# typio/entreepy

Measured on AMD Instinct MI355X. Metric: GB/s encode+decode on 1 GiB text at 1/2/4/8 MI355X; % of HBM read peak, higher is better.
Workload: dtype u8; 1 GPU; text-1G: 1073741824 B per GPU, order-0 samples of a_midsummer_nights_dream.txt's byte distribution, seed 0x5EED0004+rank, one step = encode to .et + decode back, HBM-resident; bytes_per_gpu=1073741824, packed_bytes_per_gpu=629699194

## Files before the change

entreepy_amd/csrc/et_api.cpp:

```cpp
#include <sys/stat.h>

#include "et_ctx.h"

#include <algorithm>
#include <cstdlib>
#include <vector>

namespace {

struct Geometry {
    const uint8_t *base;
    uint64_t lo, hi;
    uint32_t rpt, n_tiles;
};

Geometry make_geometry(const et_ctx *ctx, const void *d_text, size_t n) {
    Geometry g;
    const uintptr_t a = reinterpret_cast<uintptr_t>(d_text);
    g.base = reinterpret_cast<const uint8_t *>(a & ~static_cast<uintptr_t>(15));
    g.lo = a & 15;
    g.hi = g.lo + n;
    uint32_t rpt = 1;
    while (rpt < et::MAX_ROUNDS_PER_TILE && g.hi / (static_cast<uint64_t>(rpt) * et::ROUND_BYTES) > 2048) rpt <<= 1;
    if (ctx && ctx->force_rpt) rpt = ctx->force_rpt;
    g.rpt = rpt;
    const uint64_t tile_bytes = static_cast<uint64_t>(rpt) * et::ROUND_BYTES;
    g.n_tiles = static_cast<uint32_t>((g.hi + tile_bytes - 1) / tile_bytes);
    return g;
}

int ensure_encode_ws(et_ctx *ctx, uint32_t n_tiles) {
    ET_TRY(ensure(ctx, ctx->tile_hist, static_cast<size_t>(n_tiles) * 256 * sizeof(uint32_t)));
    ET_TRY(ensure(ctx, ctx->block_hist, static_cast<size_t>(et::MAX_GRID) * 256 * sizeof(uint64_t)));
    ET_TRY(ensure(ctx, ctx->hist, 256 * sizeof(uint64_t)));
    ET_TRY(ensure(ctx, ctx->tile_bits, (static_cast<size_t>(n_tiles) + 1) * sizeof(uint64_t)));
    ET_TRY(ensure(ctx, ctx->tile_off, (static_cast<size_t>(n_tiles) + 1) * sizeof(uint64_t)));
    ET_TRY(ensure(ctx, ctx->enc_table, 768 * sizeof(uint32_t) + HEADER_STAGE));
    ET_TRY(ensure(ctx, ctx->group_sum, (static_cast<size_t>(n_tiles) / 1024 + 2) * sizeof(uint64_t)));
    return ET_OK;
}

float elapsed(et_ctx *ctx, int a, int b) {
    float ms = 0.f;
    if (hipEventElapsedTime(&ms, ctx->ev[a], ctx->ev[b]) != hipSuccess) ms = 0.f;
    return ms;
}

int run_histogram(et_ctx *ctx, const void *d_text, size_t n, const Geometry &g, void *d_hist_also = nullptr) {
    ET_TRY(ensure_encode_ws(ctx, g.n_tiles));
    et::launch_hist(ctx->stream, g.base, g.lo, g.hi, g.rpt, g.n_tiles, static_cast<uint32_t *>(ctx->tile_hist.p),
                    static_cast<unsigned long long *>(ctx->block_hist.p), static_cast<unsigned long long *>(ctx->hist.p),
                    reinterpret_cast<unsigned long long *>(ctx->h_hist), ++ctx->hist_epoch, timed(ctx, 0, 1),
                    static_cast<unsigned long long *>(d_hist_also));
    ET_HIP(hipGetLastError());
    ctx->hist_text = d_text;
    ctx->hist_empty = false;
    ctx->hist_n = n;
    ctx->hist_rpt = g.rpt;
    ctx->hist_tiles = g.n_tiles;
    ctx->hist_on_host = false;
    return ET_OK;
}

int run_body(et_ctx *ctx, const et_codebook *cb, const Geometry &g, uint32_t *out32, uint64_t base_bit,
             const uint8_t *header, size_t header_len, int ev_scan, int ev_body) {
    const bool long_codes = cb->max_length > 32;
    ET_TRY(wait_for_word<uint64_t>(ctx, ctx->h_scalar + 12, ctx->enc_block_epoch, 100.0, "the code table block was never taken"));
    for (int s = 0; s < 256; ++s) {
        const uint32_t len = cb->length[s];
        uint32_t code = cb->data[s];
        if (!long_codes) code = len ? (len == 32 ? code : (code & ((1u << len) - 1u)) << (32 - len)) : 0u;
        ctx->h_enc[2 * s] = code;
        ctx->h_enc[2 * s + 1] = len;
        ctx->h_enc[512 + s] = len;
    }
    const size_t padded = (header_len + 3) & ~static_cast<size_t>(3);
    if (header_len) {
        if (padded > HEADER_STAGE) return fail(ctx, ET_ERR_ARG, "header too long");
        uint8_t *stage = reinterpret_cast<uint8_t *>(ctx->h_enc + 768);
        std::memcpy(stage, header, header_len);
        std::memset(stage + header_len, 0, padded - header_len);
    }
    et::launch_tile_scan(ctx->stream, static_cast<const uint32_t *>(ctx->tile_hist.p), g.n_tiles, cb->length, ctx->h_enc, static_cast<uint32_t *>(ctx->enc_table.p),
                         static_cast<uint32_t>(768 + padded / 4), reinterpret_cast<unsigned long long *>(ctx->h_scalar + 12), ++ctx->enc_block_epoch,
                         static_cast<unsigned long long *>(ctx->tile_bits.p),
                         static_cast<unsigned long long *>(ctx->group_sum.p), scan_epoch(ctx), base_bit,
                         static_cast<unsigned long long *>(ctx->tile_off.p), out32, static_cast<const uint32_t *>(ctx->enc_table.p) + 768,
                         static_cast<uint32_t>(padded / 4));
    ET_HIP(hipGetLastError());
    et::launch_encode(ctx->stream, g.base, g.lo, g.hi, g.rpt, g.n_tiles, static_cast<const unsigned long long *>(ctx->tile_off.p),
                      static_cast<const uint2 *>(ctx->enc_table.p), cb->max_length, out32, timed(ctx, ev_scan, ev_body));
    ET_HIP(hipGetLastError());
    return ET_OK;
}

int fetch_histogram(et_ctx *ctx) {
    if (ctx->hist_on_host) return ET_OK;
    for (uint32_t w = 0; w < et::HIST_REDUCE_GROUPS; ++w)
        ET_TRY(wait_for_word<uint64_t>(ctx, ctx->h_hist + 256 + w, ctx->hist_epoch, 100.0, "the histogram never reached the host"));
    ctx->hist_on_host = true;
    return ET_OK;
}

}

extern "C" const char *et_version(void) { return "entreepy-hip 0.1.0 (gfx950; .et format 0x01, reference v1.1.0)"; }

extern "C" const char *et_last_error(const et_ctx *ctx) { return ctx ? ctx->err.c_str() : ""; }


extern "C" int et_ctx_create(int device, et_ctx **out) {
    if (!out) return ET_ERR_ARG;
    *out = nullptr;
    int count = 0;
    if (hipGetDeviceCount(&count) != hipSuccess || device < 0 || device >= count) return ET_ERR_HIP;
    et_ctx *ctx = new (std::nothrow) et_ctx();
    if (!ctx) return ET_ERR_NOMEM;
    ctx->device = device;
    DeviceGuard guard(device);
    bool ok = guard.ok;
    ok = ok && hipStreamCreateWithFlags(&ctx->own_stream, hipStreamNonBlocking) == hipSuccess;
    ctx->stream = ctx->own_stream;
    ok = ok && hipStreamCreateWithFlags(&ctx->side.stream, hipStreamNonBlocking) == hipSuccess;
    ok = ok && hipEventCreateWithFlags(&ctx->side.fork, hipEventDisableTiming) == hipSuccess;
    ok = ok && hipEventCreateWithFlags(&ctx->side.join, hipEventDisableTiming) == hipSuccess;
    ok = ok && hipEventCreateWithFlags(&ctx->switch_ev, hipEventDisableTiming) == hipSuccess;
    ok = ok && hipHostMalloc(reinterpret_cast<void **>(&ctx->h_hist), (256 + et::HIST_REDUCE_GROUPS) * sizeof(uint64_t)) == hipSuccess;
    if (ok) std::memset(ctx->h_hist, 0, (256 + et::HIST_REDUCE_GROUPS) * sizeof(uint64_t));
    ok = ok && hipHostMalloc(reinterpret_cast<void **>(&ctx->h_enc), 768 * sizeof(uint32_t) + HEADER_STAGE) == hipSuccess;
    ok = ok && hipHostMalloc(reinterpret_cast<void **>(&ctx->h_header), HEADER_STAGE) == hipSuccess;
    for (int i = 0; i < 2; ++i) {
        ok = ok && hipHostMalloc(reinterpret_cast<void **>(&ctx->h_lut_buf[i]), DEC_TABLES_BYTES) == hipSuccess;
    }
    ctx->h_lut = ctx->h_lut_buf[0];
    ok = ok && hipHostMalloc(reinterpret_cast<void **>(&ctx->h_scalar), 16 * sizeof(uint64_t)) == hipSuccess;
    if (ok) std::memset(ctx->h_scalar, 0, 16 * sizeof(uint64_t));
    for (int i = 0; i < 2; ++i) ok = ok && hipHostMalloc(reinterpret_cast<void **>(&ctx->h_tw_tree[i]), sizeof(et::TwUpload)) == hipSuccess;
    for (auto &e : ctx->ev) ok = ok && hipEventCreateWithFlags(&e, hipEventDisableSystemFence) == hipSuccess;
    if (!ok) {
        et_ctx_destroy(ctx);
        return ET_ERR_HIP;
    }
    *out = ctx;
    return ET_OK;
}

extern "C" void et_ctx_destroy(et_ctx *ctx) {
    if (!ctx) return;
    DeviceGuard guard(ctx->device);
    (void)hipStreamSynchronize(ctx->stream);
    DevBuf *bufs[] = {&ctx->tile_hist, &ctx->block_hist, &ctx->hist, &ctx->tile_bits, &ctx->tile_off, &ctx->enc_table, &ctx->group_sum,
                      &ctx->sub_state, &ctx->blk_exit, &ctx->blk_count, &ctx->blk_off, &ctx->lut, &ctx->flag,
                      &ctx->worklist, &ctx->lane_maps, &ctx->blk_maps, &ctx->grp_maps, &ctx->blk_in, &ctx->grp_in, &ctx->row_scratch,
                      &ctx->tw_table, &ctx->tw_tree, &ctx->blk_start, &ctx->blk_pub, &ctx->chain_table, &ctx->io_in, &ctx->io_out};
    for (DevBuf *b : bufs)
        if (b->p) (void)hipFree(b->p);
    delete ctx->io;
    void *pinned[] = {ctx->h_hist, ctx->h_enc, ctx->h_header, ctx->h_lut_buf[0], ctx->h_lut_buf[1], ctx->h_scalar, ctx->h_tw_tree[0], ctx->h_tw_tree[1]};
    for (void *p : pinned)
        if (p) (void)hipHostFree(p);
    for (auto &e : ctx->ev)
        if (e) (void)hipEventDestroy(e);
    if (ctx->own_stream) (void)hipStreamDestroy(ctx->own_stream);
    if (ctx->side.stream) (void)hipStreamDestroy(ctx->side.stream);
    if (ctx->side.fork) (void)hipEventDestroy(ctx->side.fork);
    if (ctx->side.join) (void)hipEventDestroy(ctx->side.join);
    if (ctx->switch_ev) (void)hipEventDestroy(ctx->switch_ev);
    delete ctx;
}

namespace {

int switch_stream(et_ctx *ctx, hipStream_t s) {
    if (s == ctx->stream) return ET_OK;
    DeviceGuard guard(ctx->device);
    ET_HIP(hipEventRecord(ctx->switch_ev, ctx->stream));
    ET_HIP(hipStreamWaitEvent(s, ctx->switch_ev, 0));
    ctx->stream = s;
    return ET_OK;
}

}

extern "C" int et_ctx_set_stream(et_ctx *ctx, void *hip_stream) {
    if (!ctx) return ET_ERR_ARG;
    return switch_stream(ctx, static_cast<hipStream_t>(hip_stream));
}

extern "C" int et_ctx_use_own_stream(et_ctx *ctx) {
    if (!ctx) return ET_ERR_ARG;
    return switch_stream(ctx, ctx->own_stream);
}

extern "C" void *et_ctx_stream(const et_ctx *ctx) { return ctx ? static_cast<void *>(ctx->stream) : nullptr; }

extern "C" int et_ctx_device(const et_ctx *ctx) { return ctx ? ctx->device : -1; }

extern "C" int et_ctx_set_tile_rounds(et_ctx *ctx, uint32_t rounds) {
    if (!ctx) return ET_ERR_ARG;
    if (rounds > et::MAX_ROUNDS_PER_TILE || (rounds & (rounds - 1))) return ET_ERR_ARG;
    ctx->force_rpt = rounds;
    ctx->hist_text = nullptr;
    return ET_OK;
}

extern "C" int et_ctx_enable_timing(et_ctx *ctx, int on) {
    if (!ctx) return ET_ERR_ARG;
    ctx->timing = on != 0 && on != ET_TIMING_DECODE_BODY;
    ctx->timing_body = on == ET_TIMING_DECODE_BODY;
    ctx->pend_enc = ctx->pend_dec = false;
    return ET_OK;
}

extern "C" int et_last_timings_of(et_ctx *ctx, int which, et_timings *out) {
    if (!ctx || !out || which < 0 || which > 1) return ET_ERR_ARG;
    DeviceGuard guard(ctx->device);
    if (which == 0 && ctx->pend_enc) {
        ET_HIP(hipEventSynchronize(ctx->ev[3]));
        if (!ctx->pend_enc_shard) {
            ctx->tm_enc.hist_ms = elapsed(ctx, 0, 1);
            ctx->tm_enc.total_ms = elapsed(ctx, 0, 3);
        }
        ctx->tm_enc.scan_ms = ctx->pend_enc_bits ? elapsed(ctx, 1, 2) : 0.f;
        ctx->tm_enc.body_ms = elapsed(ctx, 2, 3);
        ctx->pend_enc = ctx->pend_enc_shard = false;
    }
    if (which == 1 && ctx->pend_dec && ctx->timing_body) {
        ET_HIP(hipEventSynchronize(ctx->ev[EV_DEC + 3]));
        ctx->tm_dec.body_ms = elapsed(ctx, EV_DEC + 2, EV_DEC + 3);
        ctx->pend_dec = false;
    }
    if (which == 1 && ctx->pend_dec) {
        ET_HIP(hipEventSynchronize(ctx->ev[EV_DEC + 3]));
        ctx->tm_dec.sync_ms = elapsed(ctx, EV_DEC + 0, EV_DEC + 2);
// ... 358 lines not shown
```

entreepy_amd/csrc/et_ctx.h:

```cpp
#pragma once

#include "entreepy_hip.h"

#include "et_io.h"
#include "et_kernels.h"
#include "et_rowsync.h"
#include "et_tables.h"
#include "et_treewalk.h"

#include <hip/hip_runtime.h>

#include <atomic>
#include <chrono>
#include <cstdio>
#include <cstring>
#include <string>

struct DevBuf {
    void *p = nullptr;
    size_t cap = 0;
};

constexpr size_t HEADER_STAGE = 8192;
constexpr size_t SUB_TABLE_ONLY = (static_cast<size_t>(et::DEC_SUB_TABLES_MAX) << et::DEC_SUB_BITS_MAX) * sizeof(uint16_t) + 64;
constexpr size_t SUB_TABLE_BYTES = SUB_TABLE_ONLY + 256;
constexpr size_t DEC_STEPS_OFFSET = (sizeof(uint32_t) << et::DEC_LUT_BITS_MAX) * 2 + 1024 * sizeof(uint32_t) + 2 * SUB_TABLE_BYTES;
constexpr size_t DEC_TABLES_BYTES = DEC_STEPS_OFFSET + (sizeof(uint32_t) << et::DEC_STEP_BITS_MAX) + (sizeof(uint32_t) << et::DEC_LUT_BITS_MAX) +
                                    2 * (et::DEC_STEP_SUB_WORDS + 4) * sizeof(uint32_t) + 2 * sizeof(et::DecodeTables) + sizeof(et::TablePlan) + 64;

enum class Family { TREE_WALK, WINDOWS, ROWS, FIXED_SYNC, FIXED_WRITE, EXIT_MAPS };

struct DecWs {
    uint32_t *sub_state, *blk_exit, *blk_count, *flag, *worklist;
    unsigned long long *blk_off, *group_sum;
};

struct Span : DecWs {
    const uint32_t *words;
    uint64_t n_bytes, n_subs;
    uint32_t n_blocks, first_bit;
    uint32_t tw_mode, dec_flags, row_mode;
    const et_codebook *cb;
    et::RowCode row_code;
    et::DecodeTables tb, tb_write;
    const uint16_t *tw_table;
    uint32_t tw_n_int;
    uint32_t *blk_start, *blk_pub;
    uint32_t *exit_bits;
    const uint64_t *chain;
    uint32_t n_chain;
};

struct et_ctx {
    int device = 0;
    hipStream_t own_stream = nullptr;
    et::SideLane side = {};
    hipStream_t stream = nullptr;
    hipEvent_t switch_ev = nullptr;
    bool timing = false;
    bool timing_body = false;
    uint32_t force_rpt = 0;
    uint32_t lut_bits_write = et::DEC_LUT_BITS_WRITE;
    uint32_t step_bits = et::DEC_STEP_BITS_DEFAULT;
    std::string err;

    DevBuf tile_hist, block_hist, hist, tile_bits, tile_off, enc_table, group_sum;
    DevBuf sub_state, blk_exit, blk_count, blk_off, lut, flag, worklist;
    DevBuf lane_maps, blk_maps, grp_maps, blk_in, grp_in;
    DevBuf row_scratch;
    DevBuf tw_table, tw_tree, blk_start, blk_pub, chain_table;
    et::TwUpload *h_tw_tree[2] = {};
    int tw_turn = 0;
    DevBuf io_in, io_out;
    et_io::Pipe *io = nullptr;

    uint64_t *h_hist = nullptr;
    uint32_t *h_enc = nullptr;
    uint8_t *h_header = nullptr;
    uint32_t *h_lut = nullptr;
    uint32_t *h_lut_buf[2] = {};
    int lut_turn = 0;
    uint64_t *h_scalar = nullptr;

    const void *hist_text = nullptr;
    size_t hist_n = 0;
    uint32_t hist_rpt = 0, hist_tiles = 0;
    bool hist_on_host = false;
    bool hist_empty = false;
    const void *scan_buf = nullptr;
    size_t scan_cap = 0;
    uint32_t scan_epoch_n = 0;
    uint32_t report_epoch = 0;
    uint64_t enc_block_epoch = 0;
    uint64_t header_epoch = 0;
    uint64_t hist_epoch = 0;

    hipEvent_t ev[12] = {};
    et_timings tm_enc = {}, tm_dec = {};
    bool pend_enc = false, pend_dec = false, pend_enc_bits = false, pend_enc_shard = false, pend_dec_first = false;
    int last_kind = 0;
    et_codebook last_cb = {};
    bool have_cb = false;


    struct {
        bool valid = false;
        Family family = Family::WINDOWS;
        Span s = {};
        et_codebook cb = {};
        uint64_t total = 0;
        bool maps_valid = false, maps_const = false;
    } range;
};

struct DeviceGuard {
    int prev = -1;
    bool ok = false;
    explicit DeviceGuard(int dev) {
        if (hipGetDevice(&prev) != hipSuccess) prev = -1;
        ok = hipSetDevice(dev) == hipSuccess;
    }
    ~DeviceGuard() {
        if (prev >= 0) (void)hipSetDevice(prev);
    }
};

inline int fail(et_ctx *ctx, int status, const char *what, hipError_t e = hipSuccess) {
    if (ctx) {
        ctx->err = what;
        if (e != hipSuccess) {
            ctx->err += ": ";
            ctx->err += hipGetErrorString(e);
        }
    }
    return status;
}

#define ET_HIP(call)                                                     \
    do {                                                                 \
        hipError_t e_ = (call);                                          \
        if (e_ != hipSuccess) return fail(ctx, ET_ERR_HIP, #call, e_);   \
    } while (0)

inline int ensure(et_ctx *ctx, DevBuf &b, size_t bytes) {
    if (b.cap >= bytes) return ET_OK;
    if (b.p) {
        ET_HIP(hipStreamSynchronize(ctx->stream));
        ET_HIP(hipFree(b.p));
        b.p = nullptr;
// ... 56 lines not shown
```

entreepy_amd/csrc/et_kernels.h:

```cpp
#pragma once

#include <hip/hip_runtime.h>
#include <stdint.h>

#include "et_tables.h"

#ifdef ET_GUARD_DROP_PINS
#define ET_PIN(x_) ((void)0)
#else
#define ET_PIN(x_) asm volatile("" : "+v"(x_))
#endif

namespace et {

constexpr int BLOCK = 256;
constexpr uint32_t ROUND_BYTES = BLOCK * 16;
constexpr uint32_t MAX_ROUNDS_PER_TILE = 128;
constexpr uint32_t HIST_REDUCE_GROUPS = 128;
constexpr uint32_t MAX_GRID = 2048;

constexpr uint32_t SUB_BITS = 256;
constexpr uint32_t DEC_BLOCK_WORDS = BLOCK * SUB_BITS / 32;
constexpr uint32_t DEC_GUARD_WORDS = 4;
constexpr uint32_t SYNC_CHUNK = 1, WRITE_CHUNK = 4;
constexpr bool SYNC_TICKET = false, WRITE_TICKET = true;
constexpr uint32_t DEC_FIRST_SWEEP_TRIPS = 6;
constexpr uint32_t DEC_REPAIR_SWEEP_TRIPS = 8;
__host__ __device__ inline bool dec_state_final(uint32_t gave_up, uint32_t verify_failed, uint32_t n_blocks) {
    return verify_failed == 0 && static_cast<uint64_t>(gave_up) * 64 <= n_blocks;
}
constexpr uint32_t DEC_HAVE_START = 1, DEC_FRONT_OK = 2;
constexpr uint32_t DEC_SPECIAL_SUPER = 8;
constexpr uint32_t DEC_SPECIAL_ONLY = 4;
constexpr uint32_t DEC_FRONT_WORDS = 4;
constexpr uint32_t DEC_WARMUP_BITS = DEC_FRONT_WORDS * 32;
constexpr uint32_t DEC_STAGED_WORDS = DEC_FRONT_WORDS + DEC_BLOCK_WORDS + DEC_GUARD_WORDS;
constexpr uint32_t DEC_SDATA_WORDS = (DEC_STAGED_WORDS + (DEC_STAGED_WORDS >> 5) + 4) & ~3u;
constexpr uint32_t DEC_STAGE_BYTES = 16384;

struct DecodeTables {
    const uint32_t *lut;
    const uint32_t *longc;
    const uint16_t *sub;
    const uint8_t *sym_len;
    uint32_t lut_bits;
    uint32_t n_long;
    uint32_t sub_bits;
    uint32_t n_sub;
    const uint32_t *steps;
    uint32_t step_bits;
    uint32_t step_sub_bits;
    uint32_t n_step_sub;
    const DecodeTables *dev_copy;
};

struct SideLane {
    hipStream_t stream;
    hipEvent_t fork, join;
};

struct KernelEvents {
    hipEvent_t start = nullptr, stop = nullptr;
};

void launch_hist(hipStream_t stream, const uint8_t *base, uint64_t lo, uint64_t hi, uint32_t rounds_per_tile, uint32_t n_tiles,
                 uint32_t *tile_hist, unsigned long long *block_hist, unsigned long long *hist, unsigned long long *host_hist = nullptr, unsigned long long epoch = 0,
                 KernelEvents ev = {}, unsigned long long *hist_also = nullptr);
__host__ __device__ inline uint32_t header_bound(uint8_t d) { return 8u + 6u * (static_cast<uint32_t>(d) + 1u); }
void launch_words_to_host(hipStream_t stream, const void *d_src, uint32_t n_words, void *host_dst, unsigned long long *host_done, unsigned long long epoch);
void launch_header_to_host(hipStream_t stream, const void *d_src, uint32_t n, void *host_dst, unsigned long long *host_done, unsigned long long epoch);
void launch_tile_scan(hipStream_t stream, const uint32_t *tile_hist, uint32_t n_tiles, const uint8_t *lengths, const uint32_t *host_src, uint32_t *dev_dst,
                      uint32_t copy_words, unsigned long long *host_taken, unsigned long long taken_epoch, unsigned long long *tile_bits, unsigned long long *group_sum, uint32_t epoch, unsigned long long base_bit,
                      unsigned long long *tile_off, uint32_t *out32, const uint32_t *header_src = nullptr, uint32_t header_words = 0);
void launch_encode(hipStream_t stream, const uint8_t *base, uint64_t lo, uint64_t hi, uint32_t rounds_per_tile, uint32_t n_tiles,
                   const unsigned long long *tile_off, const uint2 *enc_table, uint32_t max_len, uint32_t *out32, KernelEvents ev = {});
void launch_dec_sync(hipStream_t stream, const uint32_t *words, uint64_t n_bytes, uint32_t first_bit, uint64_t n_subs,
                     const DecodeTables &tb, uint32_t iter, uint32_t max_trips,
                     uint32_t *sub_state, uint32_t *blk_exit, uint32_t *blk_count, uint32_t *changed, uint32_t *ticket,
                     uint32_t flags = DEC_HAVE_START, uint32_t *worklist = nullptr, uint32_t *n_work = nullptr, const SideLane *side = nullptr,
                     bool ticket_is_zero = false, KernelEvents ev = {});
void launch_dec_maps(hipStream_t stream, const uint32_t *words, uint64_t n_bytes, uint32_t first_bit, bool have_start, uint64_t n_subs,
                     const DecodeTables &tb, uint32_t n_starts, uint32_t map_stride, uint8_t *lane_maps, uint8_t *blk_maps, uint8_t *grp_maps);
void launch_dec_resolve(hipStream_t stream, const uint32_t *words, uint64_t n_bytes, uint32_t first_bit, bool const_first, uint64_t n_subs,
                        const DecodeTables &tb, uint32_t map_stride, const uint8_t *lane_maps, const uint8_t *blk_maps, const uint8_t *grp_maps,
                        uint8_t *blk_in, uint8_t *grp_in, uint32_t *sub_state, uint32_t *blk_exit, uint32_t *blk_count);
void launch_dec_exhaustive(hipStream_t stream, const uint32_t *words, uint64_t n_bytes, uint32_t first_bit, uint64_t n_subs,
                           const DecodeTables &tb, uint32_t n_starts, uint32_t map_stride, uint8_t *lane_maps, uint8_t *blk_maps,
                           uint8_t *grp_maps, uint8_t *blk_in, uint8_t *grp_in, uint32_t *sub_state, uint32_t *blk_exit,
                           uint32_t *blk_count);
void launch_build_dec_tables(hipStream_t stream, const TablePlan *d_plan, uint32_t *lut, uint32_t *longc, uint16_t *sub, uint8_t *sym_len,
                             uint32_t *steps, uint32_t *wsteps, uint32_t *zero16 = nullptr);
void launch_dec_scan(hipStream_t stream, const uint32_t *blk_count, uint32_t n_blocks, unsigned long long *group_sum, uint32_t epoch,
                     unsigned long long *blk_off, unsigned long long *total_copy = nullptr, const uint32_t *verify_state = nullptr,
                     const uint32_t *verify_exit = nullptr, uint32_t *verify_flag = nullptr, uint32_t verify_first = 0xffffffffu,
                     const uint32_t *report_src = nullptr, uint32_t *report_dst = nullptr,
                     bool verify_rows = false,
                     uint32_t report_epoch = 0);
void launch_dec_write(hipStream_t stream, const uint32_t *words, uint64_t n_bytes, uint64_t n_subs, const DecodeTables &tb,
                      const uint32_t *sub_state,
                      const unsigned long long *blk_off, uint64_t n_symbols, uint8_t *out, uint32_t *ticket, const SideLane *side = nullptr,
                      bool ticket_is_zero = false, const uint32_t *void_flags = nullptr, KernelEvents ev = {},
                      const uint64_t *chain = nullptr, uint32_t n_chain = 0, uint32_t chain_max_len = 32,
                      bool strips = false);

}
```

entreepy_amd/csrc/et_kernels.hip:

```cpp
#include "et_kernels_common.h"
#include "et_treewalk.h"

namespace et {

#ifndef ET_NT_LOAD_K1
#define ET_NT_LOAD_K1 1
#endif
#ifndef ET_NT_LOAD_K4
#define ET_NT_LOAD_K4 0
#endif
#ifndef ET_NT_STORE_K4
#define ET_NT_STORE_K4 0
#endif

struct Chunk {
    uint32_t w[4];
    uint32_t valid;
};

__device__ __forceinline__ Chunk load_chunk(const uint8_t *__restrict__ base, uint64_t off, uint64_t lo, uint64_t hi) {
    Chunk c;
    if (off >= lo && off + 16 <= hi) {
        const uint4 v = *reinterpret_cast<const uint4 *>(base + off);
        c.w[0] = v.x; c.w[1] = v.y; c.w[2] = v.z; c.w[3] = v.w;
// ... 78 lines not shown
            uint4 *row = reinterpret_cast<uint4 *>(sh + tid * 32);
#pragma unroll
            for (int q = 0; q < 8; ++q) {
                const int j = (q + tid) & 7;
                const uint4 v = row[j];
                total += v.x + v.y + v.z + v.w;
                row[j] = make_uint4(0, 0, 0, 0);
            }
            tile_hist[static_cast<uint64_t>(t) * 256 + tid] = total;
            acc += total;
        }
        __syncthreads();
    }
    if (tid < 256) block_hist[static_cast<uint64_t>(tid) * HIST_ROWS + blockIdx.x] = acc;
}

__global__ __launch_bounds__(BLOCK) void k_hist_reduce(const unsigned long long *__restrict__ block_hist, uint32_t n_rows,
                                                       unsigned long long *__restrict__ hist, unsigned long long *__restrict__ host_hist,
                                                       unsigned long long epoch, unsigned long long *__restrict__ hist_also) {
    __shared__ unsigned long long part[2][4];
    const int tid = threadIdx.x, lane = tid & 63, wave = tid >> 6;
    const unsigned long long *row0 = block_hist + static_cast<uint64_t>(2 * blockIdx.x) * HIST_ROWS, *row1 = row0 + HIST_ROWS;
    unsigned long long s0 = 0, s1 = 0;
#pragma unroll
    for (uint32_t k = 0; k < HIST_ROWS / BLOCK; ++k) {
        const uint32_t r = k * BLOCK + tid;
        if (r < n_rows) {
            s0 += row0[r];
            s1 += row1[r];
        }
    }
#pragma unroll
    for (int d = 32; d >= 1; d >>= 1) {
        s0 += __shfl_xor(s0, d, 64);
        s1 += __shfl_xor(s1, d, 64);
    }
    if (lane == 0) {
        part[0][wave] = s0;
        part[1][wave] = s1;
    }
    __syncthreads();
    if (tid == 0) {
        const unsigned long long t0 = part[0][0] + part[0][1] + part[0][2] + part[0][3], t1 = part[1][0] + part[1][1] + part[1][2] + part[1][3];
        hist[2 * blockIdx.x] = t0;
        hist[2 * blockIdx.x + 1] = t1;
        if (hist_also) {
            hist_also[2 * blockIdx.x] = t0;
            hist_also[2 * blockIdx.x + 1] = t1;
        }
        if (host_hist) {
            host_hist[2 * blockIdx.x] = t0;
            host_hist[2 * blockIdx.x + 1] = t1;
            __threadfence_system();
            __hip_atomic_store(host_hist + 256 + blockIdx.x, epoch, __ATOMIC_RELEASE, __HIP_MEMORY_SCOPE_SYSTEM);
        }
    }
}

__global__ __launch_bounds__(1024) void k_header_to_host(const uint8_t *__restrict__ src, uint32_t n, uint32_t *__restrict__ host_dst,
                                                         unsigned long long *__restrict__ host_done, unsigned long long epoch) {
    const uint32_t bound = header_bound(255);
    if (bound < n) n = bound;
    for (uint32_t w = threadIdx.x; w * 4 < n; w += 1024) {
        uint32_t v = 0;
        for (uint32_t k = 0; k < 4 && w * 4 + k < n; ++k) v |= static_cast<uint32_t>(src[w * 4 + k]) << (8 * k);
        host_dst[w] = v;
    }
    __threadfence_system();
    __syncthreads();
    if (threadIdx.x == 0) __hip_atomic_store(host_done, epoch, __ATOMIC_RELEASE, __HIP_MEMORY_SCOPE_SYSTEM);
}

__global__ __launch_bounds__(1024) void k_words_to_host(const uint32_t *__restrict__ src, uint32_t n_words, uint32_t *__restrict__ host_dst,
                                                        unsigned long long *__restrict__ host_done, unsigned long long epoch) {
    for (uint32_t w = threadIdx.x; w < n_words; w += 1024) host_dst[w] = src[w];
    __threadfence_system();
    __syncthreads();
    if (threadIdx.x == 0) __hip_atomic_store(host_done, epoch, __ATOMIC_RELEASE, __HIP_MEMORY_SCOPE_SYSTEM);
}

struct CodeLengths {
    uint32_t packed[64];
};
__global__ __launch_bounds__(BLOCK) void k_tile_bits(const uint32_t *__restrict__ tile_hist, uint32_t n_tiles, const CodeLengths lengths,
                                                     unsigned long long *__restrict__ tile_bits, const uint32_t *__restrict__ host_src,
                                                     uint32_t *__restrict__ dev_dst, uint32_t copy_words, unsigned long long *__restrict__ host_taken,
                                                     unsigned long long epoch) {
    const int lane = threadIdx.x & 63;
    if (blockIdx.x == 0) {
        for (uint32_t i0 = threadIdx.x; i0 < copy_words; i0 += 8 * BLOCK) {
            uint32_t v[8];
#pragma unroll
            for (int k = 0; k < 8; ++k) v[k] = i0 + k * BLOCK < copy_words ? host_src[i0 + k * BLOCK] : 0u;
#pragma unroll
            for (int k = 0; k < 8; ++k)
                if (i0 + k * BLOCK < copy_words) dev_dst[i0 + k * BLOCK] = v[k];
        }
        __syncthreads();
        if (threadIdx.x == 0) __hip_atomic_store(host_taken, epoch, __ATOMIC_RELAXED, __HIP_MEMORY_SCOPE_SYSTEM);
    }
    const uint32_t wave_global = blockIdx.x * 4 + (threadIdx.x >> 6), n_waves = gridDim.x * 4;
    const uint32_t l4 = lengths.packed[lane];
    const uint32_t len_x = l4 & 0xffu, len_y = (l4 >> 8) & 0xffu, len_z = (l4 >> 16) & 0xffu, len_w = l4 >> 24;
    for (uint32_t t = wave_global; t < n_tiles; t += n_waves) {
        const uint4 c = reinterpret_cast<const uint4 *>(tile_hist + static_cast<uint64_t>(t) * 256)[lane];
        unsigned long long s = static_cast<unsigned long long>(c.x) * len_x + static_cast<unsigned long long>(c.y) * len_y +
                               static_cast<unsigned long long>(c.z) * len_z + static_cast<unsigned long long>(c.w) * len_w;
#pragma unroll
        for (int d = 32; d >= 1; d >>= 1) s += __shfl_xor(s, d, 64);
        if (lane == 0) tile_bits[t] = s;
    }
}

constexpr unsigned long long SCAN_TOTAL_MASK = (1ull << 47) - 1ull;
constexpr uint32_t SCAN_POLLS = 1u << 22;
template <typename T>
__global__ __launch_bounds__(1024) void k_scan_fused(const T *__restrict__ in, uint32_t n, unsigned long long *__restrict__ out,
                                                     unsigned long long *__restrict__ pub, uint32_t epoch, unsigned long long base,
                                                     uint32_t *__restrict__ zero_words, const uint32_t *__restrict__ header_src, uint32_t header_words,
                                                     unsigned long long *__restrict__ total_copy, const uint32_t *__restrict__ verify_state,
                                                     const uint32_t *__restrict__ verify_exit, uint32_t *__restrict__ verify_flag, uint32_t verify_first,
                                                     uint32_t verify_stride, uint32_t verify_mask, const uint32_t *__restrict__ report_src,
                                                     uint32_t *__restrict__ report_dst, uint32_t report_epoch) {
    __shared__ unsigned long long wsum[16], psum[16];
    __shared__ uint32_t bad_any;
    const int tid = threadIdx.x, lane = tid & 63, wave = tid >> 6;
    const uint32_t g = blockIdx.x, i = g * 1024 + tid;
    if (tid == 0) bad_any = 0;
    __syncthreads();
    if (verify_state && i < n) {
        const uint32_t want = i > 0 ? verify_exit[i - 1] : verify_first;
        if (want != 0xffffffffu && (verify_state[static_cast<uint64_t>(i) * verify_stride] & verify_mask) != want) {
            *verify_flag = 1;
            bad_any = 1;
        }
    }
    const unsigned long long x = (i < n) ? static_cast<unsigned long long>(in[i]) : 0ull;
    const unsigned long long inc = wave_inclusive_scan64(x);
    if (lane == 63) wsum[wave] = inc;
    __syncthreads();
    unsigned long long before = 0;
    for (int w = 0; w < wave; ++w) before += wsum[w];
    const unsigned long long mine = before + inc - x;
    unsigned long long group_total = 0;
    for (int w = 0; w < 16; ++w) group_total += wsum[w];
    const unsigned long long tag = static_cast<unsigned long long>(epoch) << 48;
    if (tid == 0) __hip_atomic_store(pub + g, tag | (bad_any ? 1ull << 47 : 0ull) | (group_total & SCAN_TOTAL_MASK), __ATOMIC_RELAXED, __HIP_MEMORY_SCOPE_AGENT);
    unsigned long long part = 0, bad = 0;
    for (uint32_t j = tid; j < g; j += 1024) {
        unsigned long long v = 0;
        for (uint32_t poll = 0; poll < SCAN_POLLS; ++poll) {
            v = __hip_atomic_load(pub + j, __ATOMIC_RELAXED, __HIP_MEMORY_SCOPE_AGENT);
            if ((v >> 48) == epoch) break;
            __builtin_amdgcn_s_sleep(2);
        }
        part += v & SCAN_TOTAL_MASK;
        bad |= (v >> 47) & 1ull;
    }
#pragma unroll
    for (int d = 32; d >= 1; d >>= 1) {
        part += __shfl_xor(part, d, 64);
        bad |= __shfl_xor(bad, d, 64);
    }
    if (lane == 0) psum[wave] = part | (bad << 63);
    __syncthreads();
    unsigned long long prefix = base;
    bool bad_before = false;
    for (int w = 0; w < 16; ++w) {
        prefix += psum[w] & ~(1ull << 63);
        bad_before = bad_before || (psum[w] >> 63);
    }
    const unsigned long long seam = base >> 5;
    if (i < n) {
        const unsigned long long v = mine + prefix;
        out[i] = v;
        if (zero_words && (i == 0 || ((v & 31) && (v >> 5) != seam))) zero_words[v >> 5] = 0;
    }
    if (g == gridDim.x - 1 && tid == 0) {
        const unsigned long long total = prefix + group_total;
        out[n] = total;
        if (total_copy) *total_copy = total;
        if (zero_words && (total >> 5) != seam && (total & 31)) zero_words[total >> 5] = 0;
        if (report_dst) {
            for (int k = 0; k < 12; ++k) report_dst[k] = report_src[k];
            if (verify_state) report_dst[2] = (bad_before || bad_any) ? 1u : 0u;
            report_dst[12] = static_cast<uint32_t>(total);
            report_dst[13] = static_cast<uint32_t>(total >> 32);
            __threadfence_system();
            __hip_atomic_store(report_dst + 14, report_epoch, __ATOMIC_RELEASE, __HIP_MEMORY_SCOPE_SYSTEM);
        }
    }
    if (g == 0 && header_words) {
        __syncthreads();
        for (uint32_t k = tid; k < header_words; k += 1024) zero_words[k] = header_src[k];
    }
}

struct RingFlush {
    uint32_t *ring;
    uint32_t *out32;
    bool first_word_shared;
};

template <uint32_t RING_WORDS>
__device__ __forceinline__ void flush_words(const RingFlush &f, uint32_t from, uint32_t to) {
    for (uint32_t i = from + threadIdx.x; i < to; i += BLOCK) {
        const uint32_t slot = i & (RING_WORDS - 1);
        const uint32_t v = __builtin_bswap32(f.ring[slot]);
        f.ring[slot] = 0;
        if (i == 0 && f.first_word_shared) atomicOr(f.out32, v);
#if ET_NT_STORE_K4
        else __builtin_nontemporal_store(v, f.out32 + i);
#else
        else f.out32[i] = v;
#endif
    }
}

template <uint32_t RING_WORDS>
__global__ __launch_bounds__(BLOCK) void k_encode_tiles(const uint8_t *__restrict__ base, uint64_t lo, uint64_t hi,
                                                        uint32_t rounds_per_tile, uint32_t n_tiles,
                                                        const unsigned long long *__restrict__ tile_off,
                                                        const uint2 *__restrict__ enc_table, uint32_t *__restrict__ out32) {
    __shared__ __attribute__((aligned(16))) uint32_t ring[RING_WORDS];
    __shared__ __attribute__((aligned(16))) uint2 tab[256];
    __shared__ uint32_t scratch[2][4];
    const int tid = threadIdx.x;
    tab[tid] = enc_table[tid];
    for (uint32_t i = tid; i < RING_WORDS; i += BLOCK) ring[i] = 0;
    __syncthreads();

    const uint64_t tile_bytes = static_cast<uint64_t>(rounds_per_tile) * ROUND_BYTES;
    for (uint32_t t = blockIdx.x; t < n_tiles; t += gridDim.x) {
        const unsigned long long bit0 = tile_off[t];
        RingFlush f;
        f.ring = ring;
        f.out32 = out32 + (bit0 >> 5);
        f.first_word_shared = (bit0 & 31) != 0;
        uint32_t run = static_cast<uint32_t>(bit0 & 31);
        uint32_t flushed = 0;
        const uint64_t t0 = static_cast<uint64_t>(t) * tile_bytes + static_cast<uint64_t>(tid) * 16;
        const bool interior = static_cast<uint64_t>(t) * tile_bytes >= lo && static_cast<uint64_t>(t + 1) * tile_bytes <= hi;

        Chunk cur = load_chunk_in_tile<ET_NT_LOAD_K4>(base, t0, lo, hi, interior);
#pragma unroll
        for (int k = 0; k < 4; ++k) ET_PIN(cur.w[k]);
        for (uint32_t r = 0; r < rounds_per_tile; ++r) {
            Chunk nxt;
            nxt.valid = 0;
            nxt.w[0] = nxt.w[1] = nxt.w[2] = nxt.w[3] = 0;
            if (r + 1 < rounds_per_tile) nxt = load_chunk_in_tile<ET_NT_LOAD_K4>(base, t0 + static_cast<uint64_t>(r + 1) * ROUND_BYTES, lo, hi, interior);

#define ET_ENTRY(k_) tab[(cur.w[(k_) >> 2] >> (8 * ((k_) & 3))) & 0xffu]
            uint32_t qcode[4], qlen[4];
            uint32_t tot = 0;
            bool wide4 = false;
            if (cur.valid == 0xffffu) {
#pragma unroll
                for (int q = 0; q < 4; ++q) {
                    const uint2 e0 = ET_ENTRY(4 * q), e1 = ET_ENTRY(4 * q + 1), e2 = ET_ENTRY(4 * q + 2), e3 = ET_ENTRY(4 * q + 3);
                    const uint32_t l01 = e0.y + e1.y, l23 = e2.y + e3.y;
                    const uint32_t c01 = e0.x | (e1.x >> (e0.y & 31u)), c23 = e2.x | (e3.x >> (e2.y & 31u));
                    qlen[q] = l01 + l23;
                    qcode[q] = c01 | (c23 >> (l01 & 31u));
                }
                wide4 = max(max(qlen[0], qlen[1]), max(qlen[2], qlen[3])) > 32u;
                tot = (qlen[0] + qlen[1] + qlen[2]) + qlen[3];
            } else {
                wide4 = true;
#pragma unroll
                for (int q = 0; q < 4; ++q) qcode[q] = 0, qlen[q] = 64;
                for (int k = 0; k < 16; ++k)
                    if ((cur.valid >> k) & 1u) tot += ET_ENTRY(k).y;
            }
            uint32_t round_total;
            const uint32_t excl = block_exclusive_scan(tot, scratch[r & 1], &round_total);

// ... 405 lines not shown
        walk_write_chain<2>(cw, smem8, W, start, my_lo, (win_), (win_hi_), stage_off);                     \
    }
#define WV_LDS_ORDER()                                          \
    {                                                           \
        __builtin_amdgcn_fence(__ATOMIC_RELEASE, "wavefront");  \
        __builtin_amdgcn_wave_barrier();                        \
        __builtin_amdgcn_fence(__ATOMIC_ACQUIRE, "wavefront");  \
    }
#define WV_WINDOW_STORE(win_, win_hi_)                                                                     \
    {                                                                                                      \
        WV_LDS_ORDER()                                                                                     \
        const uint32_t lo_valid = max((win_), phase);  \
        for (uint32_t g = (win_) + lane * 16; g < (win_hi_); g += 64 * 16) {                               \
            if (g >= lo_valid && g + 16 <= (win_hi_)) {                                                    \
                typedef uint32_t u32x4_nt __attribute__((ext_vector_type(4)));                             \
                 \
                __builtin_nontemporal_store(*reinterpret_cast<const u32x4_nt *>(stage + (g - (win_))), reinterpret_cast<u32x4_nt *>(out_base + g)); \
            }                                                                                              \
        }                                                                                                  \
         \
        const uint32_t head = lo_valid & ~15u, tail = (win_hi_) & ~15u;                                    \
        const uint32_t pos = (lane < 16 ? head : tail) + (lane & 15u);                                     \
        const bool partial = lane < 16 ? (lo_valid & 15u) != 0 : ((win_hi_) & 15u) != 0;  \
        if (lane < 32 && partial && pos >= lo_valid && pos < (win_hi_)) out_base[pos] = stage[pos - (win_)]; \
        WV_LDS_ORDER()                                                                                     \
    }
            uint32_t win = 0;
            bool strips_unit = false;
            if (STRIPS) strips_unit = span && !one_window && !this_edge && n_out == wave_total;
            if (strips_unit) {
                if (count) walk_write_chain<3>(cw, smem8, W, start, lds_stage + static_cast<uint32_t>(lane) * WS_STRIDE - 1u, 0, 0, 0,
#ifdef ET_PROBE_STRIPS_DENSE_DST
                                                     out + (ow & ~static_cast<uint64_t>(15)) + static_cast<uint32_t>(lane) * 64u);
#else
                                                     out + ow + my_off);
#endif
                WV_LDS_ORDER()
            } else if (span) {
                for (;; win += WV_STAGE) {
                    const uint32_t win_hi = min(win + WV_STAGE, span);
                    WV_WINDOW_WALK(win, win_hi)
                    if (win_hi == span) break;
                    WV_WINDOW_STORE(win, win_hi)
                }
            }
            WV_TAKE()
            if (span && !strips_unit) WV_WINDOW_STORE(win, span)
#undef WV_WINDOW_STORE
#undef WV_LDS_ORDER
#undef WV_WINDOW_WALK
        }
#undef WV_TAKE
#undef WV_FETCH
    }
}

template <typename K>
static uint32_t tile_grid(K kernel, uint32_t n_tiles) {
    int cus = 256;
    const int per_cu = resident_per_cu(reinterpret_cast<const void *>(kernel), 0, &cus);
    uint32_t g = per_cu >= 1 ? static_cast<uint32_t>(cus) * static_cast<uint32_t>(per_cu) : MAX_GRID;
    if (g > MAX_GRID) g = MAX_GRID;
    return n_tiles < g ? n_tiles : g;
}

void launch_hist(hipStream_t stream, const uint8_t *base, uint64_t lo, uint64_t hi, uint32_t rounds_per_tile, uint32_t n_tiles,
                 uint32_t *tile_hist, unsigned long long *block_hist, unsigned long long *hist, unsigned long long *host_hist, unsigned long long epoch, KernelEvents ev,
                 unsigned long long *hist_also) {
    const uint32_t grid = n_tiles < 1024u ? n_tiles : 1024u;
    ET_LAUNCH_TIMED(k_hist_tiles, dim3(grid), dim3(HIST_BLOCK), 0, stream, ev, base, lo, hi, rounds_per_tile, n_tiles, tile_hist, block_hist, hist);
    hipLaunchKernelGGL(k_hist_reduce, dim3(128), dim3(BLOCK), 0, stream, block_hist, grid, hist, host_hist, epoch, hist_also);
}


void launch_words_to_host(hipStream_t stream, const void *d_src, uint32_t n_words, void *host_dst, unsigned long long *host_done, unsigned long long epoch) {
    hipLaunchKernelGGL(k_words_to_host, dim3(1), dim3(1024), 0, stream, static_cast<const uint32_t *>(d_src), n_words, static_cast<uint32_t *>(host_dst), host_done, epoch);
}

void launch_header_to_host(hipStream_t stream, const void *d_src, uint32_t n, void *host_dst, unsigned long long *host_done, unsigned long long epoch) {
    hipLaunchKernelGGL(k_header_to_host, dim3(1), dim3(1024), 0, stream, static_cast<const uint8_t *>(d_src), n, static_cast<uint32_t *>(host_dst), host_done, epoch);
}

void launch_tile_scan(hipStream_t stream, const uint32_t *tile_hist, uint32_t n_tiles, const uint8_t *lengths, const uint32_t *host_src, uint32_t *dev_dst,
                      uint32_t copy_words, unsigned long long *host_taken, unsigned long long taken_epoch, unsigned long long *tile_bits, unsigned long long *group_sum, uint32_t epoch, unsigned long long base_bit,
                      unsigned long long *tile_off, uint32_t *out32, const uint32_t *header_src, uint32_t header_words) {
    uint32_t grid = (n_tiles + 3) / 4;
    if (grid > MAX_GRID) grid = MAX_GRID;
    CodeLengths cl;
    for (int l = 0; l < 64; ++l) cl.packed[l] = lengths[4 * l] | (lengths[4 * l + 1] << 8) | (lengths[4 * l + 2] << 16) | (static_cast<uint32_t>(lengths[4 * l + 3]) << 24);
    hipLaunchKernelGGL(k_tile_bits, dim3(grid), dim3(BLOCK), 0, stream, tile_hist, n_tiles, cl, tile_bits, host_src, dev_dst, copy_words, host_taken, taken_epoch);
    const uint32_t groups = (n_tiles + 1023) / 1024;
    hipLaunchKernelGGL(k_scan_fused<unsigned long long>, dim3(groups), dim3(1024), 0, stream, tile_bits, n_tiles, tile_off, group_sum, epoch, base_bit, out32, header_src,
                       header_words, static_cast<unsigned long long *>(nullptr), static_cast<const uint32_t *>(nullptr), static_cast<const uint32_t *>(nullptr),
                       static_cast<uint32_t *>(nullptr), 0xffffffffu, 0u, 0u, static_cast<const uint32_t *>(nullptr), static_cast<uint32_t *>(nullptr), 0u);
}

void launch_encode(hipStream_t stream, const uint8_t *base, uint64_t lo, uint64_t hi, uint32_t rounds_per_tile, uint32_t n_tiles,
                   const unsigned long long *tile_off, const uint2 *enc_table, uint32_t max_len, uint32_t *out32, KernelEvents ev) {
    if (max_len > 32)
        ET_LAUNCH_TIMED(k_encode_tiles_long, dim3(tile_grid(k_encode_tiles_long, n_tiles)), dim3(BLOCK), 0, stream, ev, base, lo, hi, rounds_per_tile, n_tiles, tile_off, enc_table, out32);
    else if (max_len <= 31)
        ET_LAUNCH_TIMED(k_encode_tiles<4096>, dim3(tile_grid(k_encode_tiles<4096>, n_tiles)), dim3(BLOCK), 0, stream, ev, base, lo, hi, rounds_per_tile, n_tiles, tile_off, enc_table, out32);
    else
        ET_LAUNCH_TIMED(k_encode_tiles<8192>, dim3(tile_grid(k_encode_tiles<8192>, n_tiles)), dim3(BLOCK), 0, stream, ev, base, lo, hi, rounds_per_tile, n_tiles, tile_off, enc_table, out32);
}

void launch_dec_scan(hipStream_t stream, const uint32_t *blk_count, uint32_t n_blocks, unsigned long long *group_sum, uint32_t epoch,
                     unsigned long long *blk_off, unsigned long long *total_copy, const uint32_t *verify_state, const uint32_t *verify_exit,
                     uint32_t *verify_flag, uint32_t verify_first, const uint32_t *report_src, uint32_t *report_dst, bool verify_rows, uint32_t report_epoch) {
    const uint32_t groups = (n_blocks + 1023) / 1024;
    hipLaunchKernelGGL(k_scan_fused<uint32_t>, dim3(groups), dim3(1024), 0, stream, blk_count, n_blocks, blk_off, group_sum, epoch, 0ull, static_cast<uint32_t *>(nullptr),
                       static_cast<const uint32_t *>(nullptr), 0u, total_copy, verify_state, verify_exit, verify_flag, verify_first,
                       verify_rows ? 1u : static_cast<uint32_t>(BLOCK), verify_rows ? 0xffffffffu : 0xffu, report_src, report_dst, report_epoch);
}

void launch_dec_write(hipStream_t stream, const uint32_t *words, uint64_t n_bytes, uint64_t n_subs, const DecodeTables &tb,
                      const uint32_t *sub_state,
                      const unsigned long long *blk_off, uint64_t n_symbols, uint8_t *out, uint32_t *ticket, const SideLane *side, bool ticket_is_zero,
                      const uint32_t *void_flags, KernelEvents ev, const uint64_t *chain, uint32_t n_chain, uint32_t chain_max_len, bool strips) {
    const uint32_t n_blocks = static_cast<uint32_t>((n_subs + BLOCK - 1) / BLOCK);
    if (chain) {
#ifdef ET_PROBE_FUSED_OCC
        constexpr int WAVES = ET_PROBE_FUSED_OCC;
#else
        constexpr int WAVES = 8;
#endif
        size_t smem_wave = ((static_cast<size_t>(n_chain) * 8 + 15) & ~static_cast<size_t>(15)) + WAVES * WV_STAGE_ALLOC;
#ifdef ET_PROBE_FUSED_OCC
        if (smem_wave < 84u * 1024u) smem_wave = 84u * 1024u;
#endif
        const uint32_t n_units = (n_blocks * 4 + WAVES - 1) / WAVES;
        if (strips) {
            const size_t smem_strips = ((static_cast<size_t>(n_chain) * 8 + 15) & ~static_cast<size_t>(15)) + WAVES * WS_ALLOC;
            ET_LAUNCH_TIMED((k_dec_write_wave<WAVES, true>), dim3(decode_grid(k_dec_write_wave<WAVES, true>, smem_strips, n_units, true, 64 * WAVES)), dim3(64 * WAVES), smem_strips, stream, ev, words, n_bytes, n_blocks, reinterpret_cast<const uint2 *>(chain), n_chain, sub_state, blk_off, n_symbols, out, void_flags, n_subs, chain_max_len);
            return;
        }
        ET_LAUNCH_TIMED(k_dec_write_wave<WAVES>, dim3(decode_grid(k_dec_write_wave<WAVES>, smem_wave, n_units, true, 64 * WAVES)), dim3(64 * WAVES), smem_wave, stream, ev, words, n_bytes, n_blocks, reinterpret_cast<const uint2 *>(chain), n_chain, sub_state, blk_off, n_symbols, out, void_flags, n_subs, chain_max_len);
        return;
    }
    launch_dec_write_fallback(stream, words, n_bytes, n_subs, tb, sub_state, blk_off, n_symbols, out, ticket, side, ticket_is_zero, void_flags, ev);
}


}
```

Before: 893.2 GB/s.

## Fuse tile-bit computation and prefix scan into one encode kernel

Replaces the two-kernel sequence (per-tile bit counts written to a tile_bits buffer, then a separate fused scan) with a single kernel. Each 1024-thread block computes the bit counts for 64 tiles, scans them in one wave and publishes its total. Later blocks then poll earlier blocks' published totals to build their prefix. This removes one launch and the global round trip through tile_bits. In exchange, every block polls all preceding blocks, so the work grows quadratically with block count, and correctness depends on blocks being resident while they spin.

```diff
diff --git a/entreepy_amd/csrc/et_api.cpp b/entreepy_amd/csrc/et_api.cpp
--- a/entreepy_amd/csrc/et_api.cpp
+++ b/entreepy_amd/csrc/et_api.cpp
@@ -33,10 +33,9 @@
     ET_TRY(ensure(ctx, ctx->tile_hist, static_cast<size_t>(n_tiles) * 256 * sizeof(uint32_t)));
     ET_TRY(ensure(ctx, ctx->block_hist, static_cast<size_t>(et::MAX_GRID) * 256 * sizeof(uint64_t)));
     ET_TRY(ensure(ctx, ctx->hist, 256 * sizeof(uint64_t)));
-    ET_TRY(ensure(ctx, ctx->tile_bits, (static_cast<size_t>(n_tiles) + 1) * sizeof(uint64_t)));
     ET_TRY(ensure(ctx, ctx->tile_off, (static_cast<size_t>(n_tiles) + 1) * sizeof(uint64_t)));
     ET_TRY(ensure(ctx, ctx->enc_table, 768 * sizeof(uint32_t) + HEADER_STAGE));
-    ET_TRY(ensure(ctx, ctx->group_sum, (static_cast<size_t>(n_tiles) / 1024 + 2) * sizeof(uint64_t)));
+    ET_TRY(ensure(ctx, ctx->group_sum, (static_cast<size_t>(n_tiles) / et::TILE_SCAN_TILES + 2) * sizeof(uint64_t)));
     return ET_OK;
 }
 
@@ -83,7 +82,6 @@
     }
     et::launch_tile_scan(ctx->stream, static_cast<const uint32_t *>(ctx->tile_hist.p), g.n_tiles, cb->length, ctx->h_enc, static_cast<uint32_t *>(ctx->enc_table.p),
                          static_cast<uint32_t>(768 + padded / 4), reinterpret_cast<unsigned long long *>(ctx->h_scalar + 12), ++ctx->enc_block_epoch,
-                         static_cast<unsigned long long *>(ctx->tile_bits.p),
                          static_cast<unsigned long long *>(ctx->group_sum.p), scan_epoch(ctx), base_bit,
                          static_cast<unsigned long long *>(ctx->tile_off.p), out32, static_cast<const uint32_t *>(ctx->enc_table.p) + 768,
                          static_cast<uint32_t>(padded / 4));
@@ -149,7 +147,7 @@
     if (!ctx) return;
     DeviceGuard guard(ctx->device);
     (void)hipStreamSynchronize(ctx->stream);
-    DevBuf *bufs[] = {&ctx->tile_hist, &ctx->block_hist, &ctx->hist, &ctx->tile_bits, &ctx->tile_off, &ctx->enc_table, &ctx->group_sum,
+    DevBuf *bufs[] = {&ctx->tile_hist, &ctx->block_hist, &ctx->hist, &ctx->tile_off, &ctx->enc_table, &ctx->group_sum,
                       &ctx->sub_state, &ctx->blk_exit, &ctx->blk_count, &ctx->blk_off, &ctx->lut, &ctx->flag,
                       &ctx->worklist, &ctx->lane_maps, &ctx->blk_maps, &ctx->grp_maps, &ctx->blk_in, &ctx->grp_in, &ctx->row_scratch,
                       &ctx->tw_table, &ctx->tw_tree, &ctx->blk_start, &ctx->blk_pub, &ctx->chain_table, &ctx->io_in, &ctx->io_out};
diff --git a/entreepy_amd/csrc/et_ctx.h b/entreepy_amd/csrc/et_ctx.h
--- a/entreepy_amd/csrc/et_ctx.h
+++ b/entreepy_amd/csrc/et_ctx.h
@@ -64,7 +64,7 @@
     uint32_t step_bits = et::DEC_STEP_BITS_DEFAULT;
     std::string err;
 
-    DevBuf tile_hist, block_hist, hist, tile_bits, tile_off, enc_table, group_sum;
+    DevBuf tile_hist, block_hist, hist, tile_off, enc_table, group_sum;
     DevBuf sub_state, blk_exit, blk_count, blk_off, lut, flag, worklist;
     DevBuf lane_maps, blk_maps, grp_maps, blk_in, grp_in;
     DevBuf row_scratch;
diff --git a/entreepy_amd/csrc/et_kernels.h b/entreepy_amd/csrc/et_kernels.h
--- a/entreepy_amd/csrc/et_kernels.h
+++ b/entreepy_amd/csrc/et_kernels.h
@@ -17,6 +17,7 @@
 constexpr uint32_t ROUND_BYTES = BLOCK * 16;
 constexpr uint32_t MAX_ROUNDS_PER_TILE = 128;
 constexpr uint32_t HIST_REDUCE_GROUPS = 128;
+constexpr uint32_t TILE_SCAN_TILES = 64;
 constexpr uint32_t MAX_GRID = 2048;
 
 constexpr uint32_t SUB_BITS = 256;
@@ -70,7 +71,7 @@
 void launch_words_to_host(hipStream_t stream, const void *d_src, uint32_t n_words, void *host_dst, unsigned long long *host_done, unsigned long long epoch);
 void launch_header_to_host(hipStream_t stream, const void *d_src, uint32_t n, void *host_dst, unsigned long long *host_done, unsigned long long epoch);
 void launch_tile_scan(hipStream_t stream, const uint32_t *tile_hist, uint32_t n_tiles, const uint8_t *lengths, const uint32_t *host_src, uint32_t *dev_dst,
-                      uint32_t copy_words, unsigned long long *host_taken, unsigned long long taken_epoch, unsigned long long *tile_bits, unsigned long long *group_sum, uint32_t epoch, unsigned long long base_bit,
+                      uint32_t copy_words, unsigned long long *host_taken, unsigned long long taken_epoch, unsigned long long *group_sum, uint32_t epoch, unsigned long long base_bit,
                       unsigned long long *tile_off, uint32_t *out32, const uint32_t *header_src = nullptr, uint32_t header_words = 0);
 void launch_encode(hipStream_t stream, const uint8_t *base, uint64_t lo, uint64_t hi, uint32_t rounds_per_tile, uint32_t n_tiles,
                    const unsigned long long *tile_off, const uint2 *enc_table, uint32_t max_len, uint32_t *out32, KernelEvents ev = {});
diff --git a/entreepy_amd/csrc/et_kernels.hip b/entreepy_amd/csrc/et_kernels.hip
--- a/entreepy_amd/csrc/et_kernels.hip
+++ b/entreepy_amd/csrc/et_kernels.hip
@@ -184,35 +184,6 @@
 struct CodeLengths {
     uint32_t packed[64];
 };
-__global__ __launch_bounds__(BLOCK) void k_tile_bits(const uint32_t *__restrict__ tile_hist, uint32_t n_tiles, const CodeLengths lengths,
-                                                     unsigned long long *__restrict__ tile_bits, const uint32_t *__restrict__ host_src,
-                                                     uint32_t *__restrict__ dev_dst, uint32_t copy_words, unsigned long long *__restrict__ host_taken,
-                                                     unsigned long long epoch) {
-    const int lane = threadIdx.x & 63;
-    if (blockIdx.x == 0) {
-        for (uint32_t i0 = threadIdx.x; i0 < copy_words; i0 += 8 * BLOCK) {
-            uint32_t v[8];
-#pragma unroll
-            for (int k = 0; k < 8; ++k) v[k] = i0 + k * BLOCK < copy_words ? host_src[i0 + k * BLOCK] : 0u;
-#pragma unroll
-            for (int k = 0; k < 8; ++k)
-                if (i0 + k * BLOCK < copy_words) dev_dst[i0 + k * BLOCK] = v[k];
-        }
-        __syncthreads();
-        if (threadIdx.x == 0) __hip_atomic_store(host_taken, epoch, __ATOMIC_RELAXED, __HIP_MEMORY_SCOPE_SYSTEM);
-    }
-    const uint32_t wave_global = blockIdx.x * 4 + (threadIdx.x >> 6), n_waves = gridDim.x * 4;
-    const uint32_t l4 = lengths.packed[lane];
-    const uint32_t len_x = l4 & 0xffu, len_y = (l4 >> 8) & 0xffu, len_z = (l4 >> 16) & 0xffu, len_w = l4 >> 24;
-    for (uint32_t t = wave_global; t < n_tiles; t += n_waves) {
-        const uint4 c = reinterpret_cast<const uint4 *>(tile_hist + static_cast<uint64_t>(t) * 256)[lane];
-        unsigned long long s = static_cast<unsigned long long>(c.x) * len_x + static_cast<unsigned long long>(c.y) * len_y +
-                               static_cast<unsigned long long>(c.z) * len_z + static_cast<unsigned long long>(c.w) * len_w;
-#pragma unroll
-        for (int d = 32; d >= 1; d >>= 1) s += __shfl_xor(s, d, 64);
-        if (lane == 0) tile_bits[t] = s;
-    }
-}
 
 constexpr unsigned long long SCAN_TOTAL_MASK = (1ull << 47) - 1ull;
 constexpr uint32_t SCAN_POLLS = 1u << 22;
@@ -295,6 +266,87 @@
     if (g == 0 && header_words) {
         __syncthreads();
         for (uint32_t k = tid; k < header_words; k += 1024) zero_words[k] = header_src[k];
+    }
+}
+
+__global__ __launch_bounds__(1024) void k_tile_scan(const uint32_t *__restrict__ tile_hist, uint32_t n_tiles, const CodeLengths lengths,
+                                                    const uint32_t *__restrict__ host_src, uint32_t *__restrict__ dev_dst, uint32_t copy_words,
+                                                    unsigned long long *__restrict__ host_taken, unsigned long long taken_epoch,
+                                                    unsigned long long *__restrict__ out, unsigned long long *__restrict__ pub, uint32_t epoch,
+                                                    unsigned long long base, uint32_t *__restrict__ zero_words, const uint32_t *__restrict__ header_src,
+                                                    uint32_t header_words) {
+    __shared__ unsigned long long bits[TILE_SCAN_TILES], psum[16];
+    __shared__ unsigned long long total_sh;
+    const int tid = threadIdx.x, lane = tid & 63, wave = tid >> 6;
+    const uint32_t g = blockIdx.x;
+    if (g == 0) {
+        uint32_t v[2];
+#pragma unroll
+        for (int k = 0; k < 2; ++k) v[k] = tid + k * 1024u < copy_words ? host_src[tid + k * 1024u] : 0u;
+#pragma unroll
+        for (int k = 0; k < 2; ++k)
+            if (tid + k * 1024u < copy_words) dev_dst[tid + k * 1024u] = v[k];
+        for (uint32_t i = tid + 2048; i < copy_words; i += 1024) dev_dst[i] = host_src[i];
+        __syncthreads();
+        if (tid == 0) __hip_atomic_store(host_taken, taken_epoch, __ATOMIC_RELAXED, __HIP_MEMORY_SCOPE_SYSTEM);
+    }
+    const uint32_t l4 = lengths.packed[lane];
+    const uint32_t len_x = l4 & 0xffu, len_y = (l4 >> 8) & 0xffu, len_z = (l4 >> 16) & 0xffu, len_w = l4 >> 24;
+    const uint32_t t0 = g * TILE_SCAN_TILES + wave * 4;
+    uint4 c[4];
+#pragma unroll
+    for (int k = 0; k < 4; ++k)
+        c[k] = t0 + k < n_tiles ? reinterpret_cast<const uint4 *>(tile_hist + static_cast<uint64_t>(t0 + k) * 256)[lane] : make_uint4(0, 0, 0, 0);
+#pragma unroll
+    for (int k = 0; k < 4; ++k) {
+        unsigned long long s = static_cast<unsigned long long>(c[k].x) * len_x + static_cast<unsigned long long>(c[k].y) * len_y +
+                               static_cast<unsigned long long>(c[k].z) * len_z + static_cast<unsigned long long>(c[k].w) * len_w;
+#pragma unroll
+        for (int d = 32; d >= 1; d >>= 1) s += __shfl_xor(s, d, 64);
+        if (lane == 0) bits[wave * 4 + k] = s;
+    }
+    __syncthreads();
+    unsigned long long x = 0, inc = 0;
+    if (wave == 0) {
+        x = bits[lane];
+        inc = wave_inclusive_scan64(x);
+        if (lane == 63) {
+            total_sh = inc;
+            __hip_atomic_store(pub + g, (static_cast<unsigned long long>(epoch) << 48) | (inc & SCAN_TOTAL_MASK), __ATOMIC_RELAXED, __HIP_MEMORY_SCOPE_AGENT);
+        }
+    }
+    unsigned long long part = 0;
+    for (uint32_t j = tid; j < g; j += 1024) {
+        unsigned long long v = 0;
+        for (uint32_t poll = 0; poll < SCAN_POLLS; ++poll) {
+            v = __hip_atomic_load(pub + j, __ATOMIC_RELAXED, __HIP_MEMORY_SCOPE_AGENT);
+            if ((v >> 48) == epoch) break;
+            __builtin_amdgcn_s_sleep(2);
+        }
+        part += v & SCAN_TOTAL_MASK;
+    }
+#pragma unroll
+    for (int d = 32; d >= 1; d >>= 1) part += __shfl_xor(part, d, 64);
+    if (lane == 0) psum[wave] = part;
+    __syncthreads();
+    if (wave != 0) return;
+    unsigned long long prefix = base;
+    for (int w = 0; w < 16; ++w) prefix += psum[w];
+    const unsigned long long seam = base >> 5;
+    const uint32_t i = g * TILE_SCAN_TILES + lane;
+    if (i < n_tiles) {
+        const unsigned long long v = prefix + inc - x;
+        out[i] = v;
+        if (i == 0 || ((v & 31) && (v >> 5) != seam)) zero_words[v >> 5] = 0;
+    }
+    if (g == gridDim.x - 1 && lane == 0) {
+        const unsigned long long total = prefix + total_sh;
+        out[n_tiles] = total;
+        if ((total >> 5) != seam && (total & 31)) zero_words[total >> 5] = 0;
+    }
+    if (g == 0 && header_words) {
+        asm volatile("s_waitcnt vmcnt(0)" ::: "memory");
+        for (uint32_t k = lane; k < header_words; k += 64) zero_words[k] = header_src[k];
     }
 }
 
@@ -866,17 +918,13 @@
 }
 
 void launch_tile_scan(hipStream_t stream, const uint32_t *tile_hist, uint32_t n_tiles, const uint8_t *lengths, const uint32_t *host_src, uint32_t *dev_dst,
-                      uint32_t copy_words, unsigned long long *host_taken, unsigned long long taken_epoch, unsigned long long *tile_bits, unsigned long long *group_sum, uint32_t epoch, unsigned long long base_bit,
+                      uint32_t copy_words, unsigned long long *host_taken, unsigned long long taken_epoch, unsigned long long *group_sum, uint32_t epoch, unsigned long long base_bit,
                       unsigned long long *tile_off, uint32_t *out32, const uint32_t *header_src, uint32_t header_words) {
-    uint32_t grid = (n_tiles + 3) / 4;
-    if (grid > MAX_GRID) grid = MAX_GRID;
     CodeLengths cl;
     for (int l = 0; l < 64; ++l) cl.packed[l] = lengths[4 * l] | (lengths[4 * l + 1] << 8) | (lengths[4 * l + 2] << 16) | (static_cast<uint32_t>(lengths[4 * l + 3]) << 24);
-    hipLaunchKernelGGL(k_tile_bits, dim3(grid), dim3(BLOCK), 0, stream, tile_hist, n_tiles, cl, tile_bits, host_src, dev_dst, copy_words, host_taken, taken_epoch);
-    const uint32_t groups = (n_tiles + 1023) / 1024;
-    hipLaunchKernelGGL(k_scan_fused<unsigned long long>, dim3(groups), dim3(1024), 0, stream, tile_bits, n_tiles, tile_off, group_sum, epoch, base_bit, out32, header_src,
-                       header_words, static_cast<unsigned long long *>(nullptr), static_cast<const uint32_t *>(nullptr), static_cast<const uint32_t *>(nullptr),
-                       static_cast<uint32_t *>(nullptr), 0xffffffffu, 0u, 0u, static_cast<const uint32_t *>(nullptr), static_cast<uint32_t *>(nullptr), 0u);
+    const uint32_t groups = (n_tiles + TILE_SCAN_TILES - 1) / TILE_SCAN_TILES;
+    hipLaunchKernelGGL(k_tile_scan, dim3(groups), dim3(1024), 0, stream, tile_hist, n_tiles, cl, host_src, dev_dst, copy_words, host_taken, taken_epoch, tile_off, group_sum, epoch,
+                       base_bit, out32, header_src, header_words);
 }
 
 void launch_encode(hipStream_t stream, const uint8_t *base, uint64_t lo, uint64_t hi, uint32_t rounds_per_tile, uint32_t n_tiles,
```

New measurement: 891.1 GB/s. Within noise of the previous version (-0.2%).
